# introlab/rtabmap

Hardware: AMD Instinct MI355X
Metric: loop-closure candidates/sec (49k vocab, 100k signatures, 500 desc/frame) (higher is better)
Workload: dtype f32; 1 GPU; SURF-64 fp32 brute-force 2-NN (49k words) + NNDR + TF-IDF likelihood (100000 signatures x 500 words, Zipf), 500 desc/frame, 1 frame/step; world_size_observed=1, collective_backend=none, parallelism=1 GPU, last_frame_top_candidate_ok=True

## Files before the change

### rtabmap_amd/csrc/frame_tail_body.cuh

```cuda
#pragma once
#include "tfidf.h"
#include "resolve_body.cuh"
#include "rowpar_body.cuh"

namespace lcd {
namespace {

template <typename T> __device__ __forceinline__ T gload(const T* p) { return *(const __attribute__((address_space(1))) T*)p; }
__device__ __forceinline__ uint2 gload2(const uint2* p) {
    const unsigned long long v = *(const __attribute__((address_space(1))) unsigned long long*)p;
    return make_uint2((uint32_t)v, (uint32_t)(v >> 32));
}

__device__ __forceinline__ uint4 gload4(const uint4* p) {
    typedef uint32_t u32x4 __attribute__((ext_vector_type(4)));
    const u32x4 v = *(const __attribute__((address_space(1))) u32x4*)p;
    return make_uint4(v.x, v.y, v.z, v.w);
}

__device__ __forceinline__ int32_t idf_to_fixed(float idf) {
    float s = idf * 67108864.0f;
    s = fminf(fmaxf(s, -2147483520.0f), 2147483520.0f);
    return (int32_t)rintf(s);
}
__device__ __forceinline__ float fixed_to_like(long long acc, uint32_t ni) {
    if (ni == 0u) return 0.0f;
    return __fdiv_rn(__ll2float_rn(acc) * 1.4901161193847656e-08f, (float)ni);
}

__device__ __forceinline__ void f16_split2_dev(float a, float b, uint32_t& hi, uint32_t& lo) {
    typedef _Float16 h2 __attribute__((ext_vector_type(2)));
    typedef float f2 __attribute__((ext_vector_type(2)));
    const h2 h = __builtin_convertvector((f2){a, b}, h2);
    hi = __builtin_bit_cast(uint32_t, h);
    const f2 back = __builtin_convertvector(h, f2);
    lo = __builtin_bit_cast(uint32_t, __builtin_convertvector((f2){__fsub_rn(a, back.x), __fsub_rn(b, back.y)}, h2));
}
__device__ __forceinline__ void bf16_split2_dev(float a, float b, uint32_t& hi, uint32_t& lo) {
    typedef __bf16 bf2 __attribute__((ext_vector_type(2)));
    typedef float f2 __attribute__((ext_vector_type(2)));
    hi = __builtin_bit_cast(uint32_t, __builtin_convertvector((f2){a, b}, bf2));
    const float ra = __fsub_rn(a, __uint_as_float(hi << 16)), rb = __fsub_rn(b, __uint_as_float(hi & 0xFFFF0000u));
    lo = __builtin_bit_cast(uint32_t, __builtin_convertvector((f2){ra, rb}, bf2));
}



template <int NT, bool SOLE>
__device__ __forceinline__ void frame_words_body(uint32_t* fw_smem, const FwArgs& a, const int32_t* src_lds = nullptr, bool have_ne0 = false,
                                                 uint32_t ne0 = 0u ) {
    const int H = a.H;
    uint32_t* tkey = fw_smem;
    uint32_t* tcnt = fw_smem + H;
    uint32_t* grp = tcnt + H;
    uint32_t* s_misc = grp + H / 64 + 1;
    const int tid = threadIdx.x;
    for (int i = tid; i < H; i += NT) { tkey[i] = 0xFFFFFFFFu; tcnt[i] = 0u; }
    if (tid == 0) { s_misc[0] = (SOLE && a.do_register) ? (have_ne0 ? ne0 : a.ne_counter[0]) : 0u; s_misc[1] = 0u; }
    if (have_ne0) lds_barrier(); else __syncthreads();
    for (int i = tid; i < a.n; i += NT) {
        int32_t ws = src_lds ? src_lds[i] : a.src[i];
        if (!src_lds && a.row_wslot) ws = ws >= 0 ? a.row_wslot[ws] : (ws <= -2 ? -ws - 2 : -1);
        if (a.xlate) ws = (ws > 0 && (long long)ws < a.xlate_n) ? a.xlate[ws] : -1;
        else if (ws <= -2) ws = a.new_ws.n > 0 ? ws_runs_at_dev(a.new_ws, -ws - 2) : -1;
        if (ws < 0) continue;
        const uint32_t w = (uint32_t)ws;
        uint32_t h = (w * 2654435761u) & (uint32_t)(H - 1);
        for (;;) {
            const uint32_t old = atomicCAS(&tkey[h], 0xFFFFFFFFu, w);
            if (old == 0xFFFFFFFFu || old == w) { atomicAdd(&tcnt[h], 1u); break; }
            h = (h + 1) & (uint32_t)(H - 1);
        }
    }
    lds_barrier();
    const int ng = H / 64;
    for (int i0 = 0; i0 < H; i0 += NT) {
        const int i = i0 + tid;
        const bool occ = i < H && tkey[i] != 0xFFFFFFFFu;
        const unsigned long long bal = __ballot(occ);
        if ((tid & 63) == 0 && i < H) grp[i >> 6] = (uint32_t)__popcll(bal);
    }
    lds_barrier();
    if (tid < 64) {
        uint32_t run = 0;
        for (int g0 = 0; g0 < ng; g0 += 64) {
            const int g = g0 + tid;
            const uint32_t c = g < ng ? grp[g] : 0u;
            uint32_t x = c;
#pragma unroll
            for (int off = 1; off < 64; off <<= 1) { const uint32_t y = __shfl_up(x, off, 64); if (tid >= off) x += y; }
            if (g < ng) grp[g] = run + x - c;
// ... 19 lines not shown
                u4[r] = grp[i >> 6] + (uint32_t)__popcll(bal & ((1ull << (tid & 63)) - 1ull));
                w4[r] = tkey[i];
                c4[r] = tcnt[i] > TF_CNT_MASK ? TF_CNT_MASK : tcnt[i];
            }
        }
#pragma clang diagnostic push
#pragma clang diagnostic ignored "-Wuninitialized"
#pragma clang diagnostic ignored "-Wsometimes-uninitialized"
#pragma clang diagnostic ignored "-Wconditional-uninitialized"
        const bool want_r = a.do_register && a.wrow;
#pragma unroll
        for (int r = 0; r < 4; ++r) {
            if (!o4[r]) continue;
            if (want_r) r4[r] = gload(a.wrow + w4[r]);
            if (a.do_register) n4[r] = atomicAdd(&a.nw[w4[r]], 1u);
            else n4[r] = gload(a.nw + w4[r]);
            if (a.want_q) d4[r] = gload(a.did + w4[r]);
        }
#pragma unroll
        for (int r = 0; r < 4; ++r) asm volatile("" : "+v"(n4[r]), "+v"(d4[r]), "+v"(r4[r]));
#pragma unroll
        for (int r = 0; r < 4; ++r) {
            if (!o4[r]) continue;
            const uint32_t w = w4[r], u = u4[r], cnt = c4[r], nwv = a.do_register ? n4[r] + 1u : n4[r];
            if (want_r && r4[r] == 0xFFFFFFFFu && a.q_meta) atomicAdd(&a.q_meta[8], 1u);
            if (a.do_register) {
                a.coo_w[base + u] = w;
                a.coo_pc[base + u] = (a.slot_local << TF_CNT_BITS) | cnt;
            }
            if (a.want_q) {
                float idf = 0.0f;
                if (a.N > 0.0f && nwv > 0u) idf = log10f(__fdiv_rn(a.N, (float)nwv));
                const int32_t idfq = idf_to_fixed(idf);
                const int32_t d = d4[r];
                a.q_w[u] = w;
                a.q_idf[u] = idfq;
                a.q_did[u] = d;
                a.idf_tab[w] = make_uint2(a.stamp, (uint32_t)idfq);
                if (d >= 0 && idfq != 0) {
                    const uint32_t j = atomicAdd(&s_misc[1], 1u);
                    a.qd_did[j] = d;
                    a.qd_idf[j] = idfq;
                }
            }
        }
    }
#pragma clang diagnostic pop
    lds_barrier();
    if (tid == 0) {
        if (a.want_q) { a.q_meta[0] = U; a.q_meta[1] = s_misc[1]; }
        if (a.do_register) {
            if (SOLE) a.ne_counter[0] = base + U;
            a.slot_sig[a.slot] = a.sig_id;
            a.slot_ni[a.slot] = a.ni;
            a.slot_begin[a.slot] = base;
            a.slot_cnt[a.slot] = U;
        }
    }
}


__device__ __forceinline__ void retire_body(const RetireArgs& r, const uint32_t* __restrict__ slot_begin, const uint32_t* __restrict__ slot_cnt,
                                            uint32_t* __restrict__ nw, uint32_t* __restrict__ slot_ni, int32_t* __restrict__ slot_sig) {
    for (int p = 0; p < r.n; ++p) {
        const long long slot = r.slot[p];
        const uint32_t begin = slot_begin[slot], cnt = slot_cnt[slot];
        for (uint32_t k = threadIdx.x; k < cnt; k += blockDim.x) atomicSub(&nw[r.coo_w[p][begin + k]], 1u);
        if (threadIdx.x == 0) { slot_ni[slot] = 0u; slot_sig[slot] = 0; }
    }
}
struct RetirePre { uint32_t begin[4], cnt[4]; };
__device__ __forceinline__ void retire_request(const RetireArgs& r, const uint32_t* __restrict__ slot_begin, const uint32_t* __restrict__ slot_cnt, RetirePre& pre) {
#pragma unroll
    for (int p = 0; p < 4; ++p) {
        const long long slot = p < r.n ? r.slot[p] : 0;
        pre.begin[p] = gload(slot_begin + slot); pre.cnt[p] = gload(slot_cnt + slot);
    }
}
__device__ __forceinline__ void retire_finish(const RetireArgs& r, const RetirePre& pre, uint32_t* __restrict__ nw, uint32_t* __restrict__ slot_ni,
                                              int32_t* __restrict__ slot_sig, uint32_t k_first0 = 0u ) {
    const uint32_t nt = blockDim.x;
#pragma unroll
    for (int p = 0; p < 4; ++p) {
// ... 363 lines not shown
```

### rtabmap_amd/csrc/postings_keys.h

```cpp
#pragma once
#include <map>
#include <vector>

#include "devbuf.h"
#include "lcd_kernels.h"

namespace lcd {

struct KeyIntervals {
    std::map<int32_t, int32_t> runs;
    int64_t count = 0;
    void free_key(int32_t w);
    void free_run(int32_t start, int32_t len);
    void free_verdicts(const int32_t* keys, const uint8_t* ok, size_t n);
    int take_runs(int32_t want, int max_runs, int32_t* start, int32_t* len);
    int32_t take() { int32_t s, l; return take_runs(1, 1, &s, &l) ? s : -1; }
};

struct KeyPool {
    static constexpr size_t CHECK_BATCH = 16384;
    hipStream_t stream = nullptr; int64_t* bytes_device = nullptr;
    DevBuf nw, did;
    DevBuf wrow;
    DevBuf idf_tab;
    KeyIntervals free;
    void destroy();
    hipError_t ensure_keys(int32_t n);
    int32_t n_keys() const { return n_wslots; }
    int64_t in_use() const { return (int64_t)n_wslots - free.count; }
    hipError_t key_of(int32_t word_id, bool create, int32_t* out);
    bool known(int32_t word_id) const { return (size_t)word_id < id2ws.size() && id2ws[word_id] >= 0; }
    void bind(int32_t word_id, int32_t key) {
        if ((size_t)word_id >= id2ws.size()) id2ws.resize((size_t)word_id + 1 + id2ws.size() / 2, -1);
        id2ws[word_id] = key; id2ws_dirty.push_back(word_id);
    }
    void unbind(int32_t word_id) { id2ws[word_id] = -1; id2ws_dirty.push_back(word_id); }
// ... 35 lines not shown
```

### rtabmap_amd/csrc/score_body.cuh

```cuda
#pragma once
#include "frame_tail_body.cuh"

namespace lcd {
namespace {

#ifdef LCD_SCORE_TIMING
__device__ unsigned long long g_score_timing[1024 * 8];
#define SC_STAMP(i) do { __syncthreads(); if (threadIdx.x == 0 && blockIdx.x < 1024) g_score_timing[blockIdx.x * 8 + (i)] = __builtin_amdgcn_s_memrealtime(); } while (0)
#else
#define SC_STAMP(i) do { } while (0)
#endif



template <int SCB>
__device__ __forceinline__ void score_segments(const uint32_t* __restrict__ sp_ent, unsigned long long* acc, uint32_t start, uint32_t len, int32_t idf) {
    const int ln = threadIdx.x & 63;
    uint32_t incl = len;
#pragma unroll
    for (int off = 1; off < 64; off <<= 1) { const uint32_t y = __shfl_up(incl, off, 64); if (ln >= off) incl += y; }
    const uint32_t Tw = __shfl(incl, 63, 64);
    for (uint32_t t0 = 0; t0 < Tw; t0 += 128) {
        uint32_t e[2]; int32_t f[2]; bool ok[2];
#pragma unroll
        for (int u = 0; u < 2; ++u) {
            const uint32_t t = t0 + (uint32_t)(u * 64 + ln);
            int pos = 0;
#pragma unroll
            for (int step = 32; step >= 1; step >>= 1) { const uint32_t v = __shfl(incl, pos + step - 1, 64); if (v <= t) pos += step; }
            if (pos > 63) pos = 63;
            const uint32_t i_o = __shfl(incl, pos, 64), l_o = __shfl(len, pos, 64), s_o = __shfl(start, pos, 64);
            f[u] = __shfl(idf, pos, 64);
            ok[u] = t < Tw;
            e[u] = ok[u] ? gload(sp_ent + s_o + (t - (i_o - l_o))) : 0u;
        }
#pragma unroll
        for (int u = 0; u < 2; ++u) {
            if (!ok[u]) continue;
            const long long term = (long long)(int)(e[u] & TF_CNT_MASK) * (long long)f[u];
            atomicAdd(&acc[e[u] >> TF_CNT_BITS], (unsigned long long)term);
        }
    }
}

template <int SCB>
__device__ __forceinline__ void score_sealed_body(const ScoreArgs& A, int b) {
    __shared__ unsigned long long acc[TF_R];
    const int tid = threadIdx.x;
    const BucketDev B = A.tab[b];
    const long long first_slot = (long long)b * TF_R;
    const bool live = B.state == 1u;
    SC_STAMP(0);
    constexpr int NWV = SCB / 64;
#ifndef LCD_SCORE_DR4
#define LCD_SCORE_DR4 16
#endif
    constexpr int DR = NWV == 4 ? LCD_SCORE_DR4 : (128 / NWV > 16 ? 16 : 128 / NWV);
    constexpr int KW = SCB >= 512 ? 1 : 512 / SCB;
    constexpr int NI = TF_R / SCB > 0 ? TF_R / SCB : 1;
    const int wv = __builtin_amdgcn_readfirstlane(tid >> 6), ln = tid & 63;
    const uint32_t D = live ? A.bkt_D[b] : 0u;
    const uint32_t BW = live ? B.W : 0u;
    const uint32_t flags = A.bkt_flags[b];
    const int U = (int)A.q_meta[0];
    const int Ud = (int)A.q_meta[1];
    static_assert(KW * SCB <= TF_MAX_WORDS && DR * NWV <= TF_MAX_WORDS, "the unconditional list reads stay inside the buffers");
    uint32_t w[KW]; int32_t idf[KW], did[KW]; bool look[KW];
#pragma unroll
    for (int u = 0; u < KW; ++u) {
        const int k = tid + u * SCB;
        w[u] = A.q_w[k]; idf[u] = A.q_idf[k]; did[u] = A.q_did[k];
    }
    int32_t dj[DR], fj[DR];
#pragma unroll
    for (int u = 0; u < DR; ++u) {
        const int j = wv + u * NWV;
        dj[u] = A.qd_did[j];
        fj[u] = A.qd_idf[j];
    }
#pragma unroll
    for (int u = 0; u < KW; ++u) { if (tid + u * SCB >= U) { w[u] = 0; idf[u] = 0; did[u] = -1; } }
#pragma unroll
    for (int u = 0; u < DR; ++u) { if (wv + u * NWV >= Ud) { dj[u] = -1; fj[u] = 0; } }
    uint32_t ni_v[NI];
#pragma unroll
    for (int u = 0; u < NI; ++u) { const int i = tid + u * SCB; ni_v[u] = i < TF_R ? A.slot_ni[first_slot + i] : 0u; }
    uint4 r0[KW], r1[KW];
#pragma unroll
    for (int u = 0; u < KW; ++u) {
        const bool dense_here = did[u] >= 0 && (uint32_t)did[u] < D;
        look[u] = idf[u] != 0 && w[u] < BW && (!dense_here || (flags & 1u));
        r0[u] = make_uint4(0u, 0u, 0u, 0u); r1[u] = r0[u];
        if (look[u]) {
            const uint4* rec = reinterpret_cast<const uint4*>(A.dir2 + ((size_t)(w[u] >> 5) * A.dir2_stride + (uint32_t)b) * TF_DIR2_DWORDS);
            r0[u] = gload4(rec); r1[u] = gload4(rec + 1);
        }
    }
    uint32_t c[DR];
#pragma unroll
    for (int u = 0; u < DR; ++u) c[u] = (dj[u] >= 0 && (uint32_t)dj[u] < D) ? gload((const uint32_t*)(B.dense + (size_t)dj[u] * TF_R + 4 * ln)) : 0u;
    uint32_t start[KW], len[KW];
#pragma unroll
    for (int u = 0; u < KW; ++u) {
        start[u] = 0; len[u] = 0;
        if (!look[u]) continue;
        const uint32_t f[6] = {r0[u].z, r0[u].w, r1[u].x, r1[u].y, r1[u].z, r1[u].w};
        const uint32_t p = w[u] & 31u, pd = p / 6u, ps = 5u * (p % 6u);
        if (!(r0[u].y & TF_DIR2_SAT)) {
            uint32_t before = 0;
#pragma unroll
            for (uint32_t d = 0; d < 6u; ++d) {
                const uint32_t x = d < pd ? f[d] : (d == pd ? (f[d] & ((1u << ps) - 1u)) : 0u);
                before += dir2_sum6(x);
            }
            uint32_t fd = f[0];
#pragma unroll
            for (uint32_t d = 1; d < 6u; ++d) fd = d == pd ? f[d] : fd;
            len[u] = (fd >> ps) & 31u;
            start[u] = r0[u].x + before;
        } else {
            const uint2 blk = gload2(B.dirb + (w[u] >> 5));
            const uint32_t bit = 1u << p;
            if (blk.x & bit) {
                const uint32_t r = blk.y + (uint32_t)__popc(blk.x & (bit - 1u));
                const uint32_t s0 = gload(B.sp_off + r), s1 = gload(B.sp_off + r + 1);
                start[u] = s0; len[u] = s1 - s0;
            }
        }
    }
    long long a0 = 0, a1 = 0, a2 = 0, a3 = 0;
#pragma unroll
    for (int u = 0; u < DR; ++u) {
        const long long f64 = (long long)fj[u];
        a0 += (long long)(int)(c[u] & 255u) * f64;
        a1 += (long long)(int)((c[u] >> 8) & 255u) * f64;
        a2 += (long long)(int)((c[u] >> 16) & 255u) * f64;
        a3 += (long long)(int)(c[u] >> 24) * f64;
    }
    for (int j0 = wv + DR * NWV; j0 < Ud; j0 += DR * NWV) {
#pragma unroll
        for (int u = 0; u < DR; ++u) {
            const int j = j0 + u * NWV;
            dj[u] = j < Ud ? A.qd_did[j] : -1;
            fj[u] = j < Ud ? A.qd_idf[j] : 0;
        }
#pragma unroll
        for (int u = 0; u < DR; ++u) c[u] = (dj[u] >= 0 && (uint32_t)dj[u] < D) ? gload((const uint32_t*)(B.dense + (size_t)dj[u] * TF_R + 4 * ln)) : 0u;
#pragma unroll
        for (int u = 0; u < DR; ++u) {
            const long long f64 = (long long)fj[u];
            a0 += (long long)(int)(c[u] & 255u) * f64;
            a1 += (long long)(int)((c[u] >> 8) & 255u) * f64;
            a2 += (long long)(int)((c[u] >> 16) & 255u) * f64;
            a3 += (long long)(int)(c[u] >> 24) * f64;
        }
    }
    for (int i = tid; i < TF_R; i += SCB) acc[i] = 0ull;
    __syncthreads();
    SC_STAMP(1);
    {
        const int ln4 = ln * 4;
        if (a0) atomicAdd(&acc[ln4 + 0], (unsigned long long)a0);
        if (a1) atomicAdd(&acc[ln4 + 1], (unsigned long long)a1);
        if (a2) atomicAdd(&acc[ln4 + 2], (unsigned long long)a2);
        if (a3) atomicAdd(&acc[ln4 + 3], (unsigned long long)a3);
    }
    SC_STAMP(2);
#pragma unroll
    for (int u = 0; u < KW; ++u) score_segments<SCB>(B.sp_ent, acc, start[u], len[u], idf[u]);
    for (int k0 = KW * SCB; k0 < U; k0 += SCB) {
        const int k = k0 + tid;
        uint32_t st2 = 0, ln2 = 0; int32_t idf2 = 0;
        if (k < U) {
            const uint32_t w2 = A.q_w[k];
            idf2 = A.q_idf[k];
            const int32_t d2 = A.q_did[k];
            const bool dh = d2 >= 0 && (uint32_t)d2 < D;
            if (idf2 != 0 && w2 < BW && (!dh || (flags & 1u))) {
                const uint2 bk = gload2(B.dirb + (w2 >> 5));
                const uint32_t bit = 1u << (w2 & 31);
                if (bk.x & bit) {
                    const uint32_t r = bk.y + (uint32_t)__popc(bk.x & (bit - 1u));
                    st2 = gload(B.sp_off + r);
                    ln2 = gload(B.sp_off + r + 1) - st2;
                }
            }
        }
        score_segments<SCB>(B.sp_ent, acc, st2, ln2, idf2);
// ... 56 lines not shown
```

### rtabmap_amd/csrc/similarity_body.cuh

```cuda
#pragma once
#include "frame_tail_body.cuh"

namespace lcd {
namespace {

template <int NT>
__device__ __forceinline__ void sim_query_body(uint32_t* smem, const SimQueryArgs& a) {
    const int H = a.H;
    uint32_t* tkey = smem;
    uint32_t* tcnt = smem + H;
    uint32_t* s_misc = tcnt + H;
    const int tid = threadIdx.x;
    for (int i = tid; i < H; i += NT) { tkey[i] = 0xFFFFFFFFu; tcnt[i] = 0u; }
    if (tid < 4) s_misc[tid] = 0u;
    __syncthreads();
    uint32_t valid = 0;
    for (int i = tid; i < a.n; i += NT) {
        const int32_t id = a.src[i];
        if (id <= 0) continue;
        valid += 1u;
        const int32_t ws = (long long)id < a.xlate_n ? a.xlate[id] : -1;
        if (ws < 0) continue;
        const uint32_t w = (uint32_t)ws;
        uint32_t h = (w * 2654435761u) & (uint32_t)(H - 1);
        for (;;) {
            const uint32_t old = atomicCAS(&tkey[h], 0xFFFFFFFFu, w);
            if (old == 0xFFFFFFFFu || old == w) { atomicAdd(&tcnt[h], 1u); break; }
            h = (h + 1) & (uint32_t)(H - 1);
        }
    }
#pragma unroll
    for (int off = 32; off > 0; off >>= 1) valid += __shfl_xor(valid, off, 64);
    if ((tid & 63) == 0 && valid) atomicAdd(&s_misc[2], valid);
    __syncthreads();
    for (int i0 = 0; i0 < H; i0 += NT) {
        const int i = i0 + tid;
        if (i >= H || tkey[i] == 0xFFFFFFFFu) continue;
        const uint32_t w = tkey[i], c = tcnt[i];
        const int32_t d = gload(a.did + w);
        const uint32_t u = atomicAdd(&s_misc[0], 1u);
        a.q_w[u] = w; a.q_cnt[u] = c; a.q_did[u] = d;
        a.tab[w] = make_uint2(a.stamp, c);
        if (d >= 0) {
            const uint32_t j = atomicAdd(&s_misc[1], 1u);
            a.qd_did[j] = d; a.qd_cnt[j] = c;
        }
    }
    __syncthreads();
    if (tid == 0) { a.q_meta[0] = s_misc[0]; a.q_meta[1] = s_misc[1]; a.q_meta[2] = s_misc[2]; }
}

__device__ __forceinline__ void sim_slot_nv_body(const BucketDev* __restrict__ tab, const uint32_t* __restrict__ bkt_D, int b, uint32_t* __restrict__ slot_nv) {
    __shared__ uint32_t acc[TF_R];
    const int tid = threadIdx.x, wv = tid >> 6, ln = tid & 63;
    const BucketDev B = tab[b];
    acc[tid] = 0u;
    __syncthreads();
    if (B.state == 1u) {
        const uint32_t D = min(bkt_D[b], B.D_alloc);
        uint32_t a0 = 0, a1 = 0, a2 = 0, a3 = 0;
        for (uint32_t d0 = (uint32_t)wv; d0 < D; d0 += 16u) {
            uint32_t c[4];
#pragma unroll
            for (int u = 0; u < 4; ++u) c[u] = d0 + 4u * u < D ? gload((const uint32_t*)(B.dense + (size_t)(d0 + 4u * u) * TF_R + 4 * ln)) : 0u;
#pragma unroll
            for (int u = 0; u < 4; ++u) { a0 += c[u] & 255u; a1 += (c[u] >> 8) & 255u; a2 += (c[u] >> 16) & 255u; a3 += c[u] >> 24; }
        }
        if (a0) atomicAdd(&acc[4 * ln + 0], a0);
        if (a1) atomicAdd(&acc[4 * ln + 1], a1);
        if (a2) atomicAdd(&acc[4 * ln + 2], a2);
        if (a3) atomicAdd(&acc[4 * ln + 3], a3);
        uint32_t n_sp = 0;
        if (B.W > 0u) {
            const uint2 last = gload2(B.dirb + ((B.W + 31u) / 32u - 1u));
            n_sp = gload(B.sp_off + last.y + (uint32_t)__popc(last.x));
        }
        for (uint32_t e0 = 0; e0 < n_sp; e0 += 4u * TF_R) {
            uint32_t e[4];
#pragma unroll
            for (int u = 0; u < 4; ++u) { const uint32_t i = e0 + (uint32_t)(u * TF_R + tid); e[u] = i < n_sp ? gload(B.sp_ent + i) : 0u; }
#pragma unroll
            for (int u = 0; u < 4; ++u) if (e[u] & TF_CNT_MASK) atomicAdd(&acc[e[u] >> TF_CNT_BITS], e[u] & TF_CNT_MASK);
        }
    }
    __syncthreads();
    slot_nv[(size_t)b * TF_R + tid] = acc[tid];
}

__device__ __forceinline__ void sim_write(const SimArgs& A, long long slot, uint32_t pairs, uint32_t vs, uint32_t vq, uint32_t ni) {
    const bool ok = ni != 0u && vs != 0u && vq != 0u;
    A.out_sim[slot] = ok ? __fdiv_rn((float)pairs, (float)max(vq, vs)) : 0.0f;
    if (A.out_pairs) A.out_pairs[slot] = ok ? (int32_t)pairs : 0;
    if (A.out_valid) A.out_valid[slot] = ni != 0u ? (int32_t)vs : 0;
}

__device__ __forceinline__ void sim_segments(const uint32_t* __restrict__ sp_ent, uint32_t* acc, uint32_t start, uint32_t len, uint32_t cap) {
    const int ln = threadIdx.x & 63;
    uint32_t incl = len;
#pragma unroll
    for (int off = 1; off < 64; off <<= 1) { const uint32_t y = __shfl_up(incl, off, 64); if (ln >= off) incl += y; }
    const uint32_t Tw = __shfl(incl, 63, 64);
    for (uint32_t t0 = 0; t0 < Tw; t0 += 128) {
        uint32_t e[2], f[2]; bool ok[2];
#pragma unroll
        for (int u = 0; u < 2; ++u) {
            const uint32_t t = t0 + (uint32_t)(u * 64 + ln);
            int pos = 0;
#pragma unroll
            for (int step = 32; step >= 1; step >>= 1) { const uint32_t v = __shfl(incl, pos + step - 1, 64); if (v <= t) pos += step; }
            if (pos > 63) pos = 63;
            const uint32_t i_o = __shfl(incl, pos, 64), l_o = __shfl(len, pos, 64), s_o = __shfl(start, pos, 64);
            f[u] = __shfl(cap, pos, 64);
            ok[u] = t < Tw;
            e[u] = ok[u] ? gload(sp_ent + s_o + (t - (i_o - l_o))) : 0u;
        }
#pragma unroll
        for (int u = 0; u < 2; ++u) {
            if (!ok[u]) continue;
            atomicAdd(&acc[e[u] >> TF_CNT_BITS], min(e[u] & TF_CNT_MASK, f[u]));
        }
    }
}

__device__ __forceinline__ void sim_lookup_dirb(const BucketDev& B, uint32_t w, uint32_t& start, uint32_t& len) {
    const uint2 blk = gload2(B.dirb + (w >> 5));
    const uint32_t bit = 1u << (w & 31u);
    if (blk.x & bit) {
        const uint32_t r = blk.y + (uint32_t)__popc(blk.x & (bit - 1u));
        const uint32_t s0 = gload(B.sp_off + r), s1 = gload(B.sp_off + r + 1);
        start = s0; len = s1 - s0;
    }
}

template <int SCB>
__device__ __forceinline__ void sim_sealed_body(const SimArgs& A, int b) {
    __shared__ uint32_t acc[TF_R];
    const int tid = threadIdx.x;
    const BucketDev B = A.tab[b];
    const long long first_slot = (long long)b * TF_R;
    const bool live = B.state == 1u;
    constexpr int NWV = SCB / 64;
    constexpr int DR = 128 / NWV > 16 ? 16 : 128 / NWV;
    static_assert(SCB >= 256 && SCB <= 1024 && DR * NWV <= TF_MAX_WORDS, "the unconditional list reads stay inside the buffers");
    const int wv = __builtin_amdgcn_readfirstlane(tid >> 6), ln = tid & 63;
    const uint32_t D = live ? min(A.bkt_D[b], B.D_alloc) : 0u;
    const uint32_t BW = live ? B.W : 0u;
    const uint32_t flags = A.bkt_flags[b];
    const int U = (int)A.q_meta[0];
    const int Ud = (int)A.q_meta[1];
    const uint32_t vq = A.q_meta[2];
    uint32_t w = A.q_w[tid], cq = A.q_cnt[tid]; int32_t did = A.q_did[tid];
    int32_t dj[DR]; uint32_t fj[DR];
#pragma unroll
    for (int u = 0; u < DR; ++u) {
        const int j = wv + u * NWV;
        dj[u] = A.qd_did[j];
        fj[u] = A.qd_cnt[j];
    }
    if (tid >= U) { w = 0; cq = 0; did = -1; }
#pragma unroll
    for (int u = 0; u < DR; ++u) { if (wv + u * NWV >= Ud) { dj[u] = -1; fj[u] = 0; } }
    const uint32_t ni_v = tid < TF_R ? A.slot_ni[first_slot + tid] : 0u;
    const uint32_t nv_v = tid < TF_R ? A.slot_nv[first_slot + tid] : 0u;
    const bool dense_here = did >= 0 && (uint32_t)did < D;
    const uint32_t cap = dense_here ? (cq > 255u ? cq - 255u : 0u) : cq;
    const bool look = cap != 0u && w < BW && (!dense_here || (flags & 1u));
    uint4 r0 = make_uint4(0u, 0u, 0u, 0u), r1 = r0;
    if (look) {
        const uint4* rec = reinterpret_cast<const uint4*>(A.dir2 + ((size_t)(w >> 5) * A.dir2_stride + (uint32_t)b) * TF_DIR2_DWORDS);
        r0 = gload4(rec); r1 = gload4(rec + 1);
    }
    uint32_t c[DR];
#pragma unroll
    for (int u = 0; u < DR; ++u) c[u] = (dj[u] >= 0 && (uint32_t)dj[u] < D) ? gload((const uint32_t*)(B.dense + (size_t)dj[u] * TF_R + 4 * ln)) : 0u;
    uint32_t start = 0, len = 0;
    if (look) {
        const uint32_t f[6] = {r0.z, r0.w, r1.x, r1.y, r1.z, r1.w};
        const uint32_t p = w & 31u, pd = p / 6u, ps = 5u * (p % 6u);
        if (!(r0.y & TF_DIR2_SAT)) {
            uint32_t before = 0;
#pragma unroll
            for (uint32_t d = 0; d < 6u; ++d) {
                const uint32_t x = d < pd ? f[d] : (d == pd ? (f[d] & ((1u << ps) - 1u)) : 0u);
                before += dir2_sum6(x);
            }
            uint32_t fd = f[0];
#pragma unroll
            for (uint32_t d = 1; d < 6u; ++d) fd = d == pd ? f[d] : fd;
            len = (fd >> ps) & 31u;
            start = r0.x + before;
        } else sim_lookup_dirb(B, w, start, len);
    }
    uint32_t a0 = 0, a1 = 0, a2 = 0, a3 = 0;
#pragma unroll
    for (int u = 0; u < DR; ++u) {
        a0 += min(c[u] & 255u, fj[u]); a1 += min((c[u] >> 8) & 255u, fj[u]); a2 += min((c[u] >> 16) & 255u, fj[u]); a3 += min(c[u] >> 24, fj[u]);
    }
    for (int j0 = wv + DR * NWV; j0 < Ud; j0 += DR * NWV) {
#pragma unroll
        for (int u = 0; u < DR; ++u) {
            const int j = j0 + u * NWV;
            dj[u] = j < Ud ? A.qd_did[j] : -1;
            fj[u] = j < Ud ? A.qd_cnt[j] : 0u;
        }
#pragma unroll
        for (int u = 0; u < DR; ++u) c[u] = (dj[u] >= 0 && (uint32_t)dj[u] < D) ? gload((const uint32_t*)(B.dense + (size_t)dj[u] * TF_R + 4 * ln)) : 0u;
#pragma unroll
        for (int u = 0; u < DR; ++u) {
            a0 += min(c[u] & 255u, fj[u]); a1 += min((c[u] >> 8) & 255u, fj[u]); a2 += min((c[u] >> 16) & 255u, fj[u]); a3 += min(c[u] >> 24, fj[u]);
        }
    }
    for (int i = tid; i < TF_R; i += SCB) acc[i] = 0u;
    __syncthreads();
    {
        const int ln4 = ln * 4;
        if (a0) atomicAdd(&acc[ln4 + 0], a0);
        if (a1) atomicAdd(&acc[ln4 + 1], a1);
        if (a2) atomicAdd(&acc[ln4 + 2], a2);
        if (a3) atomicAdd(&acc[ln4 + 3], a3);
    }
    sim_segments(B.sp_ent, acc, start, len, cap);
    for (int k0 = SCB; k0 < U; k0 += SCB) {
        const int k = k0 + tid;
        uint32_t st2 = 0, ln2 = 0, cap2 = 0;
        if (k < U) {
            const uint32_t w2 = A.q_w[k], cq2 = A.q_cnt[k];
            const int32_t d2 = A.q_did[k];
            const bool dh = d2 >= 0 && (uint32_t)d2 < D;
            cap2 = dh ? (cq2 > 255u ? cq2 - 255u : 0u) : cq2;
            if (cap2 != 0u && w2 < BW && (!dh || (flags & 1u))) sim_lookup_dirb(B, w2, st2, ln2);
        }
        sim_segments(B.sp_ent, acc, st2, ln2, cap2);
    }
    __syncthreads();
    if (tid < TF_R) sim_write(A, first_slot + tid, acc[tid], nv_v, vq, ni_v);
}

template <int SCB>
__device__ __forceinline__ void sim_open_body(const SimArgs& A, int ob) {
    const int wv = threadIdx.x >> 6, ln = threadIdx.x & 63;
    const int sl = ob * (SCB / 64) + wv;
    if (sl >= A.n_open_slots) return;
    const BucketDev B = A.tab[A.n_closed];
// ... 31 lines not shown
```

### rtabmap_amd/csrc/tfidf.h

```cpp
#pragma once
#include <hip/hip_runtime.h>
#include <stdint.h>
#include <unordered_map>
#include <vector>

#include "bayes.h"
#include "devbuf.h"
#include "lcd_kernels.h"
#include "postings_keys.h"

namespace lcd {

constexpr int TF_R = 256;
constexpr int TF_CNT_BITS = 22;
constexpr uint32_t TF_CNT_MASK = (1u << TF_CNT_BITS) - 1;
constexpr int TF_MAX_WORDS = 8192;
constexpr int TF_IDF_SHIFT = 26;
constexpr int TF_DENSE_T = 32;
constexpr int TF_DENSE_MAX = 4096;
constexpr int TF_DIR2_DWORDS = 8;
constexpr uint32_t TF_DIR2_SAT = 1u << 31;
__host__ __device__ inline uint32_t dir2_sum6(uint32_t x) {
    const uint32_t t = (x & 0x01F07C1Fu) + ((x >> 5) & 0x01F07C1Fu);
    return (t & 0x3FFu) + ((t >> 10) & 0x3FFu) + (t >> 20);
}

struct BucketDev {
    const uint32_t* coo_w;
    const uint32_t* coo_pc;
    const uint8_t* dense;
    const uint2* dirb;
    const uint32_t* sp_off;
    const uint32_t* sp_ent;
    uint32_t W;
    uint32_t D_alloc;
    uint32_t state;
    uint32_t pad;
};

struct SealJob {
    int bucket;
    const uint32_t* coo_w; const uint32_t* coo_pc; const uint32_t* ne;
    uint8_t* dense; uint32_t D_alloc;
    uint2* dirb; uint32_t* sp_off; uint32_t* sp_ent;
    uint32_t* dir2; uint32_t dir2_stride;
    uint32_t* cntw;
    uint32_t* tile_sums;
    uint32_t W;
    uint32_t ent_cap;
};

struct Bucket {
// ... 249 lines not shown
```

### rtabmap_amd/csrc/tfidf.hip

```cpp
#include "tfidf.h"
#include "frame_tail_body.cuh"
#include "score_body.cuh"

#include <algorithm>
#include <cmath>

namespace lcd {
namespace {

#ifndef LCD_FW_BLOCK
#define LCD_FW_BLOCK 1024
#endif
constexpr int FW_BLOCK = LCD_FW_BLOCK;
constexpr int BR_BLOCK = 256;
constexpr int SEAL_BLOCK = 256;
constexpr int SEAL_TILE = SEAL_BLOCK * 32;

template <int NT>
__device__ __forceinline__ uint32_t block_exclusive_scan(uint32_t* data, int n, uint32_t* scratch) {
    constexpr int NW = NT / 64;
    const int tid = threadIdx.x, lane = tid & 63, wv = tid >> 6;
    const int per = (n + NT - 1) / NT;
    const int lo = min(tid * per, n), hi = min(lo + per, n);
    uint32_t sum = 0;
// ... 103 lines not shown
    if (c2) atomicAdd(&cnt[2], c2);
    if (c3) atomicAdd(&cnt[3], c3);
    if (c4) atomicAdd(&cnt[4], c4);
    if (c5) atomicAdd(&cnt[5], c5);
}

__global__ void finalize_kernel(const long long* __restrict__ lfix, long long n, const uint32_t* __restrict__ slot_ni, float* __restrict__ out) {
    const long long i = (long long)blockIdx.x * blockDim.x + threadIdx.x;
    if (i < n) out[i] = fixed_to_like(lfix[i], slot_ni[i]);
}
__global__ void gather_f32_kernel(const float* __restrict__ dense, const long long* __restrict__ slots, int n, float* __restrict__ out) {
    const int i = blockIdx.x * blockDim.x + threadIdx.x;
    if (i < n) { const long long s = slots[i]; out[i] = s >= 0 ? dense[s] : 0.0f; }
}

#define SEAL_JOB() const SealJob J = jobs ? jobs[blockIdx.y] : job1

__global__ __launch_bounds__(SEAL_BLOCK) void seal_count_kernel(const SealJob* __restrict__ jobs, SealJob job1) {
    SEAL_JOB();
    const uint32_t ne = min(J.ne[0], J.ent_cap);
    for (uint32_t e = blockIdx.x * SEAL_BLOCK + threadIdx.x; e < ne; e += gridDim.x * SEAL_BLOCK) atomicAdd(&J.cntw[J.coo_w[e]], 1u);
}
__global__ __launch_bounds__(SEAL_BLOCK) void seal_densify_kernel(const SealJob* __restrict__ jobs, SealJob job1, int32_t* __restrict__ did,
                                                                  uint32_t* __restrict__ n_dense) {
    SEAL_JOB();
    for (uint32_t w = blockIdx.x * SEAL_BLOCK + threadIdx.x; w < J.W; w += gridDim.x * SEAL_BLOCK) {
        if (J.cntw[w] < (uint32_t)TF_DENSE_T || did[w] != -1) continue;
        if (__hip_atomic_load(n_dense, __ATOMIC_RELAXED, __HIP_MEMORY_SCOPE_AGENT) >= (uint32_t)TF_DENSE_MAX) continue;
        if (atomicCAS(&did[w], -1, -2) != -1) continue;
        const uint32_t id = atomicAdd(n_dense, 1u);
        did[w] = id < (uint32_t)TF_DENSE_MAX ? (int32_t)id : -1;
    }
}
__global__ __launch_bounds__(SEAL_BLOCK) void seal_classify_kernel(const SealJob* __restrict__ jobs, SealJob job1, const int32_t* __restrict__ did,
                                                                   const uint32_t* __restrict__ n_dense, uint32_t* __restrict__ bkt_D,
                                                                   uint32_t* __restrict__ bkt_flags, uint32_t* __restrict__ h_n_dense) {
    SEAL_JOB();
    const uint32_t nd = min(n_dense[0], (uint32_t)TF_DENSE_MAX);
    const uint32_t D = min(nd, J.D_alloc);
    if (blockIdx.x == 0 && threadIdx.x == 0) { bkt_D[J.bucket] = D; if (h_n_dense && blockIdx.y == 0) h_n_dense[0] = nd; }
    const uint32_t ne = min(J.ne[0], J.ent_cap);
    for (uint32_t e = blockIdx.x * SEAL_BLOCK + threadIdx.x; e < ne; e += gridDim.x * SEAL_BLOCK) {
        const uint32_t w = J.coo_w[e], pc = J.coo_pc[e];
        const int32_t d = did[w];
        if (d < 0 || (uint32_t)d >= D) continue;
        const uint32_t cnt = pc & TF_CNT_MASK, sl = pc >> TF_CNT_BITS;
        J.dense[(size_t)d * TF_R + sl] = (uint8_t)min(cnt, 255u);
        if (cnt <= 255u) atomicSub(&J.cntw[w], 1u);
        else atomicOr(&bkt_flags[J.bucket], 1u);
    }
}
__global__ __launch_bounds__(SEAL_BLOCK) void seal_tile_kernel(const SealJob* __restrict__ jobs, SealJob job1) {
    SEAL_JOB();
    __shared__ uint32_t s_p[SEAL_BLOCK / 64], s_a[SEAL_BLOCK / 64];
    const uint32_t w0 = (blockIdx.x * SEAL_BLOCK + threadIdx.x) * 32u;
    uint32_t p = 0, a = 0;
    for (uint32_t i = 0; i < 32u && w0 + i < J.W; ++i) { const uint32_t c = J.cntw[w0 + i]; p += c ? 1u : 0u; a += c; }
#pragma unroll
    for (int off = 32; off > 0; off >>= 1) { p += __shfl_xor(p, off, 64); a += __shfl_xor(a, off, 64); }
    if ((threadIdx.x & 63) == 0) { s_p[threadIdx.x >> 6] = p; s_a[threadIdx.x >> 6] = a; }
    __syncthreads();
    if (threadIdx.x == 0) {
        uint32_t tp = 0, ta = 0;
        for (int i = 0; i < SEAL_BLOCK / 64; ++i) { tp += s_p[i]; ta += s_a[i]; }
        J.tile_sums[2 * blockIdx.x] = tp; J.tile_sums[2 * blockIdx.x + 1] = ta;
    }
}
__global__ __launch_bounds__(SEAL_BLOCK) void seal_scan_kernel(const SealJob* __restrict__ jobs, SealJob job1) {
    SEAL_JOB();
    __shared__ uint32_t s_p[SEAL_BLOCK], s_a[SEAL_BLOCK], scratch[SEAL_BLOCK / 64 + 1];
    uint32_t base_p = 0, base_a = 0;
    for (uint32_t t = 0; t < blockIdx.x; ++t) { base_p += J.tile_sums[2 * t]; base_a += J.tile_sums[2 * t + 1]; }
    const uint32_t blk = blockIdx.x * SEAL_BLOCK + threadIdx.x;
    const uint32_t w0 = blk * 32u;
    uint32_t bits = 0, p = 0, a = 0;
    uint32_t c[32];
#pragma unroll
    for (uint32_t i = 0; i < 32u; ++i) {
        c[i] = (w0 + i < J.W) ? J.cntw[w0 + i] : 0u;
        if (c[i]) { bits |= 1u << i; p += 1u; }
        a += c[i];
    }
    s_p[threadIdx.x] = p; s_a[threadIdx.x] = a;
    __syncthreads();
    const uint32_t tot_p = block_exclusive_scan<SEAL_BLOCK>(s_p, SEAL_BLOCK, scratch);
    const uint32_t tot_a = block_exclusive_scan<SEAL_BLOCK>(s_a, SEAL_BLOCK, scratch);
    uint32_t rp = base_p + s_p[threadIdx.x], ra = base_a + s_a[threadIdx.x];
    if (w0 < J.W) {
        J.dirb[blk] = make_uint2(bits, rp);
        if (J.dir2) {
            uint32_t f[6] = {0u, 0u, 0u, 0u, 0u, 0u};
            bool sat = false;
#pragma unroll
            for (uint32_t i = 0; i < 32u; ++i) { sat = sat || c[i] > 30u; f[i / 6] |= (c[i] > 30u ? 31u : c[i]) << (5u * (i % 6)); }
            uint4* rec = reinterpret_cast<uint4*>(J.dir2 + ((size_t)blk * J.dir2_stride + (uint32_t)J.bucket) * TF_DIR2_DWORDS);
            rec[0] = make_uint4(ra, rp | (sat ? TF_DIR2_SAT : 0u), f[0], f[1]);
            rec[1] = make_uint4(f[2], f[3], f[4], f[5]);
        }
    }
#pragma unroll
    for (uint32_t i = 0; i < 32u; ++i) if (c[i]) { J.sp_off[rp++] = ra; ra += c[i]; }
    if (blockIdx.x == gridDim.x - 1 && threadIdx.x == 0) J.sp_off[base_p + tot_p] = base_a + tot_a;
}
__global__ __launch_bounds__(SEAL_BLOCK) void seal_scatter_kernel(const SealJob* __restrict__ jobs, SealJob job1, const int32_t* __restrict__ did,
                                                                  const uint32_t* __restrict__ bkt_D) {
    SEAL_JOB();
    const uint32_t D = bkt_D[J.bucket];
    const uint32_t ne = min(J.ne[0], J.ent_cap);
    for (uint32_t e = blockIdx.x * SEAL_BLOCK + threadIdx.x; e < ne; e += gridDim.x * SEAL_BLOCK) {
        const uint32_t w = J.coo_w[e];
        uint32_t pc = J.coo_pc[e];
        const int32_t d = did[w];
        if (d >= 0 && (uint32_t)d < D) {
            const uint32_t cnt = pc & TF_CNT_MASK;
            if (cnt <= 255u) continue;
            pc = (pc & ~TF_CNT_MASK) | (cnt - 255u);
        }
        const uint2 blk = J.dirb[w >> 5];
        const uint32_t r = blk.y + (uint32_t)__popc(blk.x & ((1u << (w & 31)) - 1u));
        const uint32_t pos = J.sp_off[r] + atomicSub(&J.cntw[w], 1u) - 1u;
        J.sp_ent[pos] = pc;
    }
}

__global__ void set_bucket_kernel(BucketDev* tab, int b, BucketDev v) { tab[b] = v; }

__global__ void retire_kernel(long long slot, const uint32_t* __restrict__ coo_w, const uint32_t* __restrict__ slot_begin,
                              const uint32_t* __restrict__ slot_cnt, uint32_t* __restrict__ nw, uint32_t* __restrict__ slot_ni,
                              int32_t* __restrict__ slot_sig) {
    const uint32_t begin = slot_begin[slot], cnt = slot_cnt[slot];
    for (uint32_t k = threadIdx.x; k < cnt; k += blockDim.x) atomicSub(&nw[coo_w[begin + k]], 1u);
    if (threadIdx.x == 0) { slot_ni[slot] = 0u; slot_sig[slot] = 0; }
}

inline int next_pow2(int v) { int p = 2; while (p < v) p <<= 1; return p; }

}

__device__ __forceinline__ int shard_owned_below(int32_t id, int32_t first, int32_t block, int rank, int world) {
    if (id <= first) return 0;
    const long long x = (long long)id - first, cyc = (long long)block * world;
    const long long rem = x % cyc - (long long)rank * block;
    return (int)((x / cyc) * block + (rem < 0 ? 0 : (rem > block ? block : rem)));
}
__device__ __forceinline__ void shard_append_body(int* s_first , const AppendArgs& ap,
// ... 556 lines not shown
```

Baseline: 3.922 billion candidates/s.

## Split dense tile cells into low/high nibble halves with heavy-word list

Dense per-signature count cells are repacked from one byte per slot into two nibble planes: a low-nibble half that is always read and a high-nibble half read only for words flagged heavy (count >= 16). A heavy flag bit is folded into the did value and a separate heavy query list is built, so the scoring and similarity kernels read 16-bit instead of 32-bit words per lane for most dense words. This halves dense-row traffic in the common case, at the cost of atomicOr-based sealing, an extra list pass, and flag decoding everywhere did is used.

```diff
diff --git a/rtabmap_amd/csrc/dense_cells.h b/rtabmap_amd/csrc/dense_cells.h
--- /dev/null
+++ b/rtabmap_amd/csrc/dense_cells.h
@@ -0,0 +1,27 @@
+#pragma once
+#include <stdint.h>
+
+#if defined(__HIPCC__) || defined(__CUDACC__)
+#define LCD_HD __host__ __device__
+#else
+#define LCD_HD
+#endif
+
+namespace lcd {
+
+constexpr int DENSE_HALF_BYTES = 128;
+constexpr int DENSE_HALF_DWORDS = DENSE_HALF_BYTES / 4;
+constexpr uint32_t DENSE_HEAVY_MIN = 16;
+
+constexpr int32_t DID_HEAVY = 1 << 16;
+LCD_HD inline int32_t did_id(int32_t v) { return v < 0 ? v : (v & (DID_HEAVY - 1)); }
+LCD_HD inline bool did_heavy(int32_t v) { return v >= 0 && (v & DID_HEAVY) != 0; }
+
+LCD_HD inline uint32_t dense_cell_dword(uint32_t sl) { return sl >> 3; }
+LCD_HD inline uint32_t dense_cell_shift(uint32_t sl) { return 4u * (sl & 7u); }
+LCD_HD inline uint32_t dense_cell_lo_bits(uint32_t cell, uint32_t sl) { return (cell & 15u) << dense_cell_shift(sl); }
+LCD_HD inline uint32_t dense_cell_hi_bits(uint32_t cell, uint32_t sl) { return (cell >> 4) << dense_cell_shift(sl); }
+LCD_HD inline uint32_t dense_nibble(uint32_t h16, int k) { return (h16 >> (4 * k)) & 15u; }
+LCD_HD inline uint32_t dense_cell(uint32_t lo16, uint32_t hi16, int k) { return dense_nibble(lo16, k) | (dense_nibble(hi16, k) << 4); }
+
+}
diff --git a/rtabmap_amd/csrc/frame_tail_body.cuh b/rtabmap_amd/csrc/frame_tail_body.cuh
--- a/rtabmap_amd/csrc/frame_tail_body.cuh
+++ b/rtabmap_amd/csrc/frame_tail_body.cuh
@@ -56,7 +56,7 @@
     uint32_t* s_misc = grp + H / 64 + 1;
     const int tid = threadIdx.x;
     for (int i = tid; i < H; i += NT) { tkey[i] = 0xFFFFFFFFu; tcnt[i] = 0u; }
-    if (tid == 0) { s_misc[0] = (SOLE && a.do_register) ? (have_ne0 ? ne0 : a.ne_counter[0]) : 0u; s_misc[1] = 0u; }
+    if (tid == 0) { s_misc[0] = (SOLE && a.do_register) ? (have_ne0 ? ne0 : a.ne_counter[0]) : 0u; s_misc[1] = 0u; s_misc[2] = 0u; }
     if (have_ne0) lds_barrier(); else __syncthreads();
     for (int i = tid; i < a.n; i += NT) {
         int32_t ws = src_lds ? src_lds[i] : a.src[i];
@@ -142,7 +142,7 @@
                 float idf = 0.0f;
                 if (a.N > 0.0f && nwv > 0u) idf = log10f(__fdiv_rn(a.N, (float)nwv));
                 const int32_t idfq = idf_to_fixed(idf);
-                const int32_t d = d4[r];
+                const int32_t d = did_id(d4[r]);
                 a.q_w[u] = w;
                 a.q_idf[u] = idfq;
                 a.q_did[u] = d;
@@ -151,6 +151,11 @@
                     const uint32_t j = atomicAdd(&s_misc[1], 1u);
                     a.qd_did[j] = d;
                     a.qd_idf[j] = idfq;
+                    if (did_heavy(d4[r])) {
+                        const uint32_t jh = atomicAdd(&s_misc[2], 1u);
+                        a.qd_did[TF_HEAVY_LIST + jh] = d;
+                        a.qd_idf[TF_HEAVY_LIST + jh] = idfq;
+                    }
                 }
             }
         }
@@ -158,7 +163,7 @@
 #pragma clang diagnostic pop
     lds_barrier();
     if (tid == 0) {
-        if (a.want_q) { a.q_meta[0] = U; a.q_meta[1] = s_misc[1]; }
+        if (a.want_q) { a.q_meta[0] = U; a.q_meta[1] = s_misc[1]; a.q_meta[2] = s_misc[2]; }
         if (a.do_register) {
             if (SOLE) a.ne_counter[0] = base + U;
             a.slot_sig[a.slot] = a.sig_id;
diff --git a/rtabmap_amd/csrc/postings_keys.h b/rtabmap_amd/csrc/postings_keys.h
--- a/rtabmap_amd/csrc/postings_keys.h
+++ b/rtabmap_amd/csrc/postings_keys.h
@@ -2,6 +2,7 @@
 #include <map>
 #include <vector>
 
+#include "dense_cells.h"
 #include "devbuf.h"
 #include "lcd_kernels.h"
 
diff --git a/rtabmap_amd/csrc/score_body.cuh b/rtabmap_amd/csrc/score_body.cuh
--- a/rtabmap_amd/csrc/score_body.cuh
+++ b/rtabmap_amd/csrc/score_body.cuh
@@ -12,6 +12,16 @@
 #endif
 
 
+
+__device__ __forceinline__ uint32_t dense_half_load(const uint8_t* dense, int32_t d, uint32_t D, int half, int ln) {
+    return (d >= 0 && (uint32_t)d < D) ? (uint32_t)gload((const uint16_t*)(dense + (size_t)d * TF_R + half * DENSE_HALF_BYTES + 2 * ln)) : 0u;
+}
+__device__ __forceinline__ void dense_half_add(uint32_t h, long long f64, long long& a0, long long& a1, long long& a2, long long& a3) {
+    a0 += (long long)(int)dense_nibble(h, 0) * f64;
+    a1 += (long long)(int)dense_nibble(h, 1) * f64;
+    a2 += (long long)(int)dense_nibble(h, 2) * f64;
+    a3 += (long long)(int)dense_nibble(h, 3) * f64;
+}
 
 template <int SCB>
 __device__ __forceinline__ void score_segments(const uint32_t* __restrict__ sp_ent, unsigned long long* acc, uint32_t start, uint32_t len, int32_t idf) {
@@ -56,6 +66,7 @@
 #define LCD_SCORE_DR4 16
 #endif
     constexpr int DR = NWV == 4 ? LCD_SCORE_DR4 : (128 / NWV > 16 ? 16 : 128 / NWV);
+    constexpr int HR = NWV >= 8 ? 1 : 8 / NWV;
     constexpr int KW = SCB >= 512 ? 1 : 512 / SCB;
     constexpr int NI = TF_R / SCB > 0 ? TF_R / SCB : 1;
     const int wv = __builtin_amdgcn_readfirstlane(tid >> 6), ln = tid & 63;
@@ -64,7 +75,8 @@
     const uint32_t flags = A.bkt_flags[b];
     const int U = (int)A.q_meta[0];
     const int Ud = (int)A.q_meta[1];
-    static_assert(KW * SCB <= TF_MAX_WORDS && DR * NWV <= TF_MAX_WORDS, "the unconditional list reads stay inside the buffers");
+    const int Uh = (int)A.q_meta[2];
+    static_assert(KW * SCB <= TF_MAX_WORDS && DR * NWV <= TF_MAX_WORDS && TF_HEAVY_LIST + HR * NWV <= TF_MAX_WORDS, "the unconditional list reads stay inside the buffers");
     uint32_t w[KW]; int32_t idf[KW], did[KW]; bool look[KW];
 #pragma unroll
     for (int u = 0; u < KW; ++u) {
@@ -78,10 +90,19 @@
         dj[u] = A.qd_did[j];
         fj[u] = A.qd_idf[j];
     }
+    int32_t hd[HR], hf[HR];
+#pragma unroll
+    for (int u = 0; u < HR; ++u) {
+        const int j = TF_HEAVY_LIST + wv + u * NWV;
+        hd[u] = A.qd_did[j];
+        hf[u] = A.qd_idf[j];
+    }
 #pragma unroll
     for (int u = 0; u < KW; ++u) { if (tid + u * SCB >= U) { w[u] = 0; idf[u] = 0; did[u] = -1; } }
 #pragma unroll
     for (int u = 0; u < DR; ++u) { if (wv + u * NWV >= Ud) { dj[u] = -1; fj[u] = 0; } }
+#pragma unroll
+    for (int u = 0; u < HR; ++u) { if (wv + u * NWV >= Uh) { hd[u] = -1; hf[u] = 0; } }
     uint32_t ni_v[NI];
 #pragma unroll
     for (int u = 0; u < NI; ++u) { const int i = tid + u * SCB; ni_v[u] = i < TF_R ? A.slot_ni[first_slot + i] : 0u; }
@@ -96,9 +117,12 @@
             r0[u] = gload4(rec); r1[u] = gload4(rec + 1);
         }
     }
+    uint32_t ch[HR];
+#pragma unroll
+    for (int u = 0; u < HR; ++u) ch[u] = dense_half_load(B.dense, hd[u], D, 1, ln);
     uint32_t c[DR];
 #pragma unroll
-    for (int u = 0; u < DR; ++u) c[u] = (dj[u] >= 0 && (uint32_t)dj[u] < D) ? gload((const uint32_t*)(B.dense + (size_t)dj[u] * TF_R + 4 * ln)) : 0u;
+    for (int u = 0; u < DR; ++u) c[u] = dense_half_load(B.dense, dj[u], D, 0, ln);
     uint32_t start[KW], len[KW];
 #pragma unroll
     for (int u = 0; u < KW; ++u) {
@@ -130,13 +154,9 @@
     }
     long long a0 = 0, a1 = 0, a2 = 0, a3 = 0;
 #pragma unroll
-    for (int u = 0; u < DR; ++u) {
-        const long long f64 = (long long)fj[u];
-        a0 += (long long)(int)(c[u] & 255u) * f64;
-        a1 += (long long)(int)((c[u] >> 8) & 255u) * f64;
-        a2 += (long long)(int)((c[u] >> 16) & 255u) * f64;
-        a3 += (long long)(int)(c[u] >> 24) * f64;
-    }
+    for (int u = 0; u < HR; ++u) dense_half_add(ch[u], (long long)hf[u] * 16, a0, a1, a2, a3);
+#pragma unroll
+    for (int u = 0; u < DR; ++u) dense_half_add(c[u], (long long)fj[u], a0, a1, a2, a3);
     for (int j0 = wv + DR * NWV; j0 < Ud; j0 += DR * NWV) {
 #pragma unroll
         for (int u = 0; u < DR; ++u) {
@@ -145,15 +165,21 @@
             fj[u] = j < Ud ? A.qd_idf[j] : 0;
         }
 #pragma unroll
-        for (int u = 0; u < DR; ++u) c[u] = (dj[u] >= 0 && (uint32_t)dj[u] < D) ? gload((const uint32_t*)(B.dense + (size_t)dj[u] * TF_R + 4 * ln)) : 0u;
-#pragma unroll
-        for (int u = 0; u < DR; ++u) {
-            const long long f64 = (long long)fj[u];
-            a0 += (long long)(int)(c[u] & 255u) * f64;
-            a1 += (long long)(int)((c[u] >> 8) & 255u) * f64;
-            a2 += (long long)(int)((c[u] >> 16) & 255u) * f64;
-            a3 += (long long)(int)(c[u] >> 24) * f64;
-        }
+        for (int u = 0; u < DR; ++u) c[u] = dense_half_load(B.dense, dj[u], D, 0, ln);
+#pragma unroll
+        for (int u = 0; u < DR; ++u) dense_half_add(c[u], (long long)fj[u], a0, a1, a2, a3);
+    }
+    for (int j0 = wv + HR * NWV; j0 < Uh; j0 += HR * NWV) {
+#pragma unroll
+        for (int u = 0; u < HR; ++u) {
+            const int j = j0 + u * NWV;
+            hd[u] = j < Uh ? A.qd_did[TF_HEAVY_LIST + j] : -1;
+            hf[u] = j < Uh ? A.qd_idf[TF_HEAVY_LIST + j] : 0;
+        }
+#pragma unroll
+        for (int u = 0; u < HR; ++u) ch[u] = dense_half_load(B.dense, hd[u], D, 1, ln);
+#pragma unroll
+        for (int u = 0; u < HR; ++u) dense_half_add(ch[u], (long long)hf[u] * 16, a0, a1, a2, a3);
     }
     for (int i = tid; i < TF_R; i += SCB) acc[i] = 0ull;
     __syncthreads();
diff --git a/rtabmap_amd/csrc/similarity_body.cuh b/rtabmap_amd/csrc/similarity_body.cuh
--- a/rtabmap_amd/csrc/similarity_body.cuh
+++ b/rtabmap_amd/csrc/similarity_body.cuh
@@ -39,7 +39,7 @@
         const uint32_t w = tkey[i], c = tcnt[i];
         const int32_t d = gload(a.did + w);
         const uint32_t u = atomicAdd(&s_misc[0], 1u);
-        a.q_w[u] = w; a.q_cnt[u] = c; a.q_did[u] = d;
+        a.q_w[u] = w; a.q_cnt[u] = c; a.q_did[u] = did_id(d);
         a.tab[w] = make_uint2(a.stamp, c);
         if (d >= 0) {
             const uint32_t j = atomicAdd(&s_misc[1], 1u);
@@ -60,11 +60,15 @@
         const uint32_t D = min(bkt_D[b], B.D_alloc);
         uint32_t a0 = 0, a1 = 0, a2 = 0, a3 = 0;
         for (uint32_t d0 = (uint32_t)wv; d0 < D; d0 += 16u) {
-            uint32_t c[4];
-#pragma unroll
-            for (int u = 0; u < 4; ++u) c[u] = d0 + 4u * u < D ? gload((const uint32_t*)(B.dense + (size_t)(d0 + 4u * u) * TF_R + 4 * ln)) : 0u;
-#pragma unroll
-            for (int u = 0; u < 4; ++u) { a0 += c[u] & 255u; a1 += (c[u] >> 8) & 255u; a2 += (c[u] >> 16) & 255u; a3 += c[u] >> 24; }
+            uint32_t c[4], ch[4];
+#pragma unroll
+            for (int u = 0; u < 4; ++u) {
+                const uint8_t* row = B.dense + (size_t)(d0 + 4u * u) * TF_R + 2 * ln;
+                c[u] = d0 + 4u * u < D ? (uint32_t)gload((const uint16_t*)row) : 0u;
+                ch[u] = d0 + 4u * u < D ? (uint32_t)gload((const uint16_t*)(row + DENSE_HALF_BYTES)) : 0u;
+            }
+#pragma unroll
+            for (int u = 0; u < 4; ++u) { a0 += dense_cell(c[u], ch[u], 0); a1 += dense_cell(c[u], ch[u], 1); a2 += dense_cell(c[u], ch[u], 2); a3 += dense_cell(c[u], ch[u], 3); }
         }
         if (a0) atomicAdd(&acc[4 * ln + 0], a0);
         if (a1) atomicAdd(&acc[4 * ln + 1], a1);
@@ -130,6 +134,14 @@
         const uint32_t s0 = gload(B.sp_off + r), s1 = gload(B.sp_off + r + 1);
         start = s0; len = s1 - s0;
     }
+}
+
+__device__ __forceinline__ uint32_t sim_half_load(const uint8_t* dense, int32_t dv, uint32_t D, int half, int ln) {
+    const int32_t d = did_id(dv);
+    return (d >= 0 && (uint32_t)d < D) ? (uint32_t)gload((const uint16_t*)(dense + (size_t)d * TF_R + half * DENSE_HALF_BYTES + 2 * ln)) : 0u;
+}
+__device__ __forceinline__ void sim_cells_add(uint32_t lo, uint32_t hi, uint32_t cq, uint32_t& a0, uint32_t& a1, uint32_t& a2, uint32_t& a3) {
+    a0 += min(dense_cell(lo, hi, 0), cq); a1 += min(dense_cell(lo, hi, 1), cq); a2 += min(dense_cell(lo, hi, 2), cq); a3 += min(dense_cell(lo, hi, 3), cq);
 }
 
 template <int SCB>
@@ -170,9 +182,9 @@
         const uint4* rec = reinterpret_cast<const uint4*>(A.dir2 + ((size_t)(w >> 5) * A.dir2_stride + (uint32_t)b) * TF_DIR2_DWORDS);
         r0 = gload4(rec); r1 = gload4(rec + 1);
     }
-    uint32_t c[DR];
-#pragma unroll
-    for (int u = 0; u < DR; ++u) c[u] = (dj[u] >= 0 && (uint32_t)dj[u] < D) ? gload((const uint32_t*)(B.dense + (size_t)dj[u] * TF_R + 4 * ln)) : 0u;
+    uint32_t c[DR], ch[DR];
+#pragma unroll
+    for (int u = 0; u < DR; ++u) { c[u] = sim_half_load(B.dense, dj[u], D, 0, ln); ch[u] = did_heavy(dj[u]) ? sim_half_load(B.dense, dj[u], D, 1, ln) : 0u; }
     uint32_t start = 0, len = 0;
     if (look) {
         const uint32_t f[6] = {r0.z, r0.w, r1.x, r1.y, r1.z, r1.w};
@@ -193,9 +205,7 @@
     }
     uint32_t a0 = 0, a1 = 0, a2 = 0, a3 = 0;
 #pragma unroll
-    for (int u = 0; u < DR; ++u) {
-        a0 += min(c[u] & 255u, fj[u]); a1 += min((c[u] >> 8) & 255u, fj[u]); a2 += min((c[u] >> 16) & 255u, fj[u]); a3 += min(c[u] >> 24, fj[u]);
-    }
+    for (int u = 0; u < DR; ++u) sim_cells_add(c[u], ch[u], fj[u], a0, a1, a2, a3);
     for (int j0 = wv + DR * NWV; j0 < Ud; j0 += DR * NWV) {
 #pragma unroll
         for (int u = 0; u < DR; ++u) {
@@ -204,11 +214,9 @@
             fj[u] = j < Ud ? A.qd_cnt[j] : 0u;
         }
 #pragma unroll
-        for (int u = 0; u < DR; ++u) c[u] = (dj[u] >= 0 && (uint32_t)dj[u] < D) ? gload((const uint32_t*)(B.dense + (size_t)dj[u] * TF_R + 4 * ln)) : 0u;
-#pragma unroll
-        for (int u = 0; u < DR; ++u) {
-            a0 += min(c[u] & 255u, fj[u]); a1 += min((c[u] >> 8) & 255u, fj[u]); a2 += min((c[u] >> 16) & 255u, fj[u]); a3 += min(c[u] >> 24, fj[u]);
-        }
+        for (int u = 0; u < DR; ++u) { c[u] = sim_half_load(B.dense, dj[u], D, 0, ln); ch[u] = did_heavy(dj[u]) ? sim_half_load(B.dense, dj[u], D, 1, ln) : 0u; }
+#pragma unroll
+        for (int u = 0; u < DR; ++u) sim_cells_add(c[u], ch[u], fj[u], a0, a1, a2, a3);
     }
     for (int i = tid; i < TF_R; i += SCB) acc[i] = 0u;
     __syncthreads();
diff --git a/rtabmap_amd/csrc/tfidf.h b/rtabmap_amd/csrc/tfidf.h
--- a/rtabmap_amd/csrc/tfidf.h
+++ b/rtabmap_amd/csrc/tfidf.h
@@ -18,6 +18,8 @@
 constexpr int TF_IDF_SHIFT = 26;
 constexpr int TF_DENSE_T = 32;
 constexpr int TF_DENSE_MAX = 4096;
+constexpr int TF_HEAVY_LIST = TF_DENSE_MAX;
+static_assert(DID_HEAVY > TF_DENSE_MAX, "a dense id fits below the heavy flag");
 constexpr int TF_DIR2_DWORDS = 8;
 constexpr uint32_t TF_DIR2_SAT = 1u << 31;
 __host__ __device__ inline uint32_t dir2_sum6(uint32_t x) {
diff --git a/rtabmap_amd/csrc/tfidf.hip b/rtabmap_amd/csrc/tfidf.hip
--- a/rtabmap_amd/csrc/tfidf.hip
+++ b/rtabmap_amd/csrc/tfidf.hip
@@ -159,7 +159,7 @@
         did[w] = id < (uint32_t)TF_DENSE_MAX ? (int32_t)id : -1;
     }
 }
-__global__ __launch_bounds__(SEAL_BLOCK) void seal_classify_kernel(const SealJob* __restrict__ jobs, SealJob job1, const int32_t* __restrict__ did,
+__global__ __launch_bounds__(SEAL_BLOCK) void seal_classify_kernel(const SealJob* __restrict__ jobs, SealJob job1, int32_t* __restrict__ did,
                                                                    const uint32_t* __restrict__ n_dense, uint32_t* __restrict__ bkt_D,
                                                                    uint32_t* __restrict__ bkt_flags, uint32_t* __restrict__ h_n_dense) {
     SEAL_JOB();
@@ -169,10 +169,16 @@
     const uint32_t ne = min(J.ne[0], J.ent_cap);
     for (uint32_t e = blockIdx.x * SEAL_BLOCK + threadIdx.x; e < ne; e += gridDim.x * SEAL_BLOCK) {
         const uint32_t w = J.coo_w[e], pc = J.coo_pc[e];
-        const int32_t d = did[w];
+        const int32_t dv = did[w], d = did_id(dv);
         if (d < 0 || (uint32_t)d >= D) continue;
         const uint32_t cnt = pc & TF_CNT_MASK, sl = pc >> TF_CNT_BITS;
-        J.dense[(size_t)d * TF_R + sl] = (uint8_t)min(cnt, 255u);
+        const uint32_t cell = min(cnt, 255u);
+        uint32_t* row = reinterpret_cast<uint32_t*>(J.dense + (size_t)d * TF_R) + dense_cell_dword(sl);
+        if (cell & 15u) atomicOr(row, dense_cell_lo_bits(cell, sl));
+        if (cell >= DENSE_HEAVY_MIN) {
+            atomicOr(row + DENSE_HALF_DWORDS, dense_cell_hi_bits(cell, sl));
+            if (!(dv & DID_HEAVY)) atomicOr(&did[w], DID_HEAVY);
+        }
         if (cnt <= 255u) atomicSub(&J.cntw[w], 1u);
         else atomicOr(&bkt_flags[J.bucket], 1u);
     }
@@ -237,7 +243,7 @@
     for (uint32_t e = blockIdx.x * SEAL_BLOCK + threadIdx.x; e < ne; e += gridDim.x * SEAL_BLOCK) {
         const uint32_t w = J.coo_w[e];
         uint32_t pc = J.coo_pc[e];
-        const int32_t d = did[w];
+        const int32_t d = did_id(did[w]);
         if (d >= 0 && (uint32_t)d < D) {
             const uint32_t cnt = pc & TF_CNT_MASK;
             if (cnt <= 255u) continue;
```

After: 3.842 billion candidates/s. -2.0%, worse.
